# ThatTanishqTak/3D-Renderer

Hardware: AMD Instinct MI355X
Metric: frames/sec + Mpixels/sec at 1080p & 4K; achieved HBM GB/s vs roofline (higher is better)
Workload: dtype f32; 1 GPU; c3_grid1m_3840x2160; width=3840, height=2160, triangles=999698, vertices=501264, bin=32, skybox=reference Trident-Forge/Assets/Skyboxes PNG faces (512^2, assets/Skyboxes), frames_in_flight=3, parallelism=single GPU

## Files before the change

3d-renderer_amd/csrc/raster_bin.h:

```cpp
#pragma once
#include "raster_device.h"

#ifndef TRI_PK_SHADE
#error "raster_bin.h: define TRI_PK_SHADE (0 or 1) before the include"
#endif

#ifndef TRI_BIG_AREA
#define TRI_BIG_AREA 96
#endif
#ifndef TRI_BIG_AREA16
#define TRI_BIG_AREA16 160
#endif
#ifndef TRI_RASTER_PRIO
#define TRI_RASTER_PRIO 0
#endif
#ifndef TRI_QTAB_BIGN
#define TRI_QTAB_BIGN 192
#endif

namespace {

constexpr uint64_t kBgKey = 0x3F800001ull << 32;
constexpr float kPi = 3.14159265359f;

// ... 204 lines not shown
    cx0 = max(-floor_shift8(128 - xmin), ox);
    cx1 = min(floor_shift8(xmax - 128), ox + bw - 1);
    cy0 = max(-floor_shift8(128 - ymin), oy);
    cy1 = min(floor_shift8(ymax - 128), oy + bh - 1);
}

__device__ __forceinline__ uint32_t key_low(uint32_t prim_sub) {
    return ((TRI_PRIM_MAX - (prim_sub >> 3)) << 3) | (prim_sub & 7u);
}

constexpr uint32_t kQtab = 256, kQPrimMax = (1u << 20) - 1u;
__device__ __forceinline__ uint32_t qenc(uint32_t prim_sub, uint32_t qpos) {
    const uint32_t low = ((kQPrimMax - (prim_sub >> 3)) << 11) | ((prim_sub & 7u) << 8) | qpos;
    return (TRI_PRIM_MAX - (low >> 3)) << 3 | (low & 7u);
}

__device__ __forceinline__ bool edge_start(const TriRec& r, int32_t cx0, int32_t cy0, int32_t A[3], int32_t B[3],
                                          int32_t F[3], float& dzdX, float& dzdY) {
    const int32_t xmin = min(r.X[0], min(r.X[1], r.X[2])), xmax = max(r.X[0], max(r.X[1], r.X[2]));
    const int32_t ymin = min(r.Y[0], min(r.Y[1], r.Y[2])), ymax = max(r.Y[0], max(r.Y[1], r.Y[2]));
    if (xmax - xmin < 16384 && ymax - ymin < 16384) {
        const int32_t Xc = 256 * cx0 + 128, Yc = 256 * cy0 + 128;
#pragma unroll
        for (int k = 0; k < 3; ++k) {
            const int i = k, j = (k + 1) % 3;
            const int32_t a = r.Y[i] - r.Y[j];
            const int32_t bb = r.X[j] - r.X[i];
            const bool tl = (a > 0) || (a == 0 && bb > 0);
            A[k] = a;
            B[k] = bb;
// ... 697 lines not shown
    const uint4 &st = sh.st, &sd = sh.sd, &ss = sh.ss;
    TriTexDesc td;
    td.texels = reinterpret_cast<const uint32_t*>(((uint64_t)sd.y << 32) | sd.x);
    td.w = sd.z; td.h = sd.w;
    td.solid[0] = __uint_as_float(ss.x); td.solid[1] = __uint_as_float(ss.y);
    td.solid[2] = __uint_as_float(ss.z); td.solid[3] = __uint_as_float(ss.w);
    const float4 tx = (kAblate & 128) ? make_float4(u, v, u, 1.0f) : sample_tex(td, u, v, lut);
    const float4 tint = make_float4(__uint_as_float(st.x), __uint_as_float(st.y), __uint_as_float(st.z), __uint_as_float(st.w));
    put(11, tx.x); put(12, tx.y); put(13, tx.z); put(14, tx.w);
    put(15, tint.x); put(16, tint.y); put(17, tint.z); put(18, tint.w);
}

template <bool EXACT, bool SHADOW, bool ONE, int CLIPM = 0, int KIND = kKindGeneric, typename Put>
__device__ __forceinline__ void fetch_fragment_to(const TriFrameParams& fp, const TriDeviceBuffers& b, uint64_t key,
                                                  int32_t px, int32_t py, const float* lut, Put&& put,
                                                  const uint32_t* qtab = nullptr, const FetchBufs* fbk = nullptr) {
    constexpr bool kInlineVis = SHADOW;
    const uint32_t low = (uint32_t)key;
    const uint32_t prim = qtab ? kQPrimMax - (low >> 11) : TRI_PRIM_MAX - (low >> 3);
    const uint32_t sub = CLIPM == 1 ? 0u : (qtab ? (low >> 8) & 7u : low & 7u);
    const FetchBufs fb = (KIND >= 0 && fbk) ? *fbk : fetch_bufs<ONE, KIND>(fp, b);
    constexpr bool kEarly = ONE && !EXACT && !SHADOW;
    const bool ucol = ONE && kind_flag<KIND>(TRI_KIND_UCOL, obj_mode(fp) && fp.obj_ucol);
    const bool vcol = KIND >= 0 ? !ucol : (kEarly || !ucol);
    uint32_t sl[3] = {0, 0, 0}, d = 0;
    TriSnap a0{}, a1{}, a2{};
    uint32_t v0 = 0, v1 = 0, v2 = 0, dl = 0;
    Taps taps;
    if (CLIPM != 2) {
        if (qtab) {
            const uint32_t q = low & 0xFFu;
            sl[0] = qtab[q]; sl[1] = qtab[kQtab + q]; sl[2] = qtab[2 * kQtab + q];
            if (!ONE) d = qtab[3 * kQtab + q];
        } else {
            prim_slots<ONE, !SHADOW>(fp, b, prim, sl, d);
// ... 41 lines not shown

    float vis = 1.0f;
    if constexpr (kInlineVis && !(kAblate & 2048)) {
        auto ix = [&](uint32_t a, uint32_t bq, uint32_t c) {
            return interp_exact(w0, w1, w2, __uint_as_float(a), __uint_as_float(bq), __uint_as_float(c));
        };
        vis = shadow_vis(fp, b.shadow_map, ix(L0.x, L1.x, L2.x), ix(L0.y, L1.y, L2.y), ix(L0.z, L1.z, L2.z));
    }
    put(19, vis);
    fetch_attrs<EXACT, ONE, !SHADOW, KIND>(fp, b, fb, taps, d, w0, w1, w2, lut, put);
}

template <bool EXACT, bool SHADOW, bool ONE, int CLIPM = 0, int KIND = kKindGeneric>
__device__ __forceinline__ void fetch_fragment(const TriFrameParams& fp, const TriDeviceBuffers& b, uint64_t key,
                                               int32_t px, int32_t py, const float* lut, Frag& f,
                                               const uint32_t* qtab = nullptr, const FetchBufs* fbk = nullptr) {
    fetch_fragment_to<EXACT, SHADOW, ONE, CLIPM, KIND>(fp, b, key, px, py, lut, [&](int i, float x) { (&f.wx)[i] = x; },
                                                       qtab, fbk);
}

template <bool FAST = false>
__device__ __forceinline__ int cube_face(f3 d, float& s, float& t) {
    const float ax = fabsf(d.x), ay = fabsf(d.y), az = fabsf(d.z);
    int face;
    float ma, sc, tc;
    if (ax >= ay && ax >= az) {
        face = d.x >= 0.0f ? 0 : 1; ma = ax; sc = d.x >= 0.0f ? -d.z : d.z; tc = -d.y;
    } else if (ay >= az) {
        face = d.y >= 0.0f ? 2 : 3; ma = ay; sc = d.x; tc = d.y >= 0.0f ? d.z : -d.z;
    } else {
        face = d.z >= 0.0f ? 4 : 5; ma = az; sc = d.z >= 0.0f ? d.x : -d.x; tc = -d.y;
    }
    if (!(ma > 0.0f)) { s = 0.5f; t = 0.5f; return face; }
// ... 213 lines not shown
        const float w = fp.ai_wgt;
        const float alpha = ONE ? fp.sc.sbt[3] : c.w;
        if (fs_fast_nan(fp.sc, f)) return unorm8(mix_ai(alpha, ai.w, w)) << 24;
        return fast_bgra(mix_ai(c.x, 255.0f * ai.x, w), mix_ai(c.y, 255.0f * ai.y, w), mix_ai(c.z, 255.0f * ai.z, w),
                         unorm8(mix_ai(alpha, ai.w, w)));
    }
    return fast_bgra(c.x, c.y, c.z, ONE ? a8 : unorm8(c.w));
}

template <bool EXACT, int BL, bool SHADOW, bool ONE = false, bool AI = false, int KIND = kKindGeneric>
__device__ __forceinline__ void raster_bin(const TriFrameParams& fp, const TriDeviceBuffers& b, const int bin) {
    constexpr int BIN = 1 << BL;
    __shared__ uint64_t keys[BIN * BIN];
    constexpr bool kBalanced = BL == 4;
    constexpr bool kQt = BL == 5 && (ONE || SHADOW);
    constexpr uint32_t kQw = ONE ? 3u : 4u;
    constexpr int kBigN = kBalanced ? kBigQueue / 2 : ((kQt && ONE) ? TRI_QTAB_BIGN : kBigQueue);
    __shared__ uint32_t bigq[kBigN];
    __shared__ float lut[512];
    constexpr int kJobWords = (kBalanced && kCovJobs > BIN * BIN ? kCovJobs : BIN * BIN);
    __shared__ uint16_t skyq[kJobWords];
    __shared__ CovEntry cov[kBalanced ? kCovPass : 1];
    __shared__ uint32_t wsum[TRI_BLOCK / 64];
    __shared__ uint32_t nbig, nsky;
    __shared__ uint32_t qtab[kQt ? kQw * kQtab : 1];
    __shared__ uint16_t bigqp[kQt ? kBigN : 1];
    const int tid = threadIdx.x;
    TRI_STAMP(0);
    if constexpr (BL == 5) __builtin_amdgcn_s_setprio(1 + TRI_RASTER_PRIO);
    const int bx = bin % fp.nbx, by = bin / fp.nbx;
    const int32_t ox = bx * BIN, oy = fp.y0 + by * BIN;
    const int32_t bw = min(BIN, fp.W - ox), bh = min(BIN, fp.y1 - oy);
    const uint32_t cnt_v = __builtin_amdgcn_raw_buffer_load_b32(make_rsrc(b.bin_count, 4ull * fp.nbins), (uint32_t)bin * 4u, 0, 0);
    uint32_t pre1 = 0;
    if constexpr (!kBalanced) {
        const Rsrc qr = make_rsrc(b.bin_list + (size_t)bin * fp.bin_cap, 4ull * fp.bin_cap);
        pre1 = __builtin_amdgcn_raw_buffer_load_b32(qr, (uint32_t)tid * 4u, 0, 0);
    }
    for (int i = tid; i < BIN * BIN; i += TRI_BLOCK) keys[i] = kBgKey;
    if (fp.need_lut)
        for (int i = tid; i < 512; i += TRI_BLOCK) lut[i] = b.srgb_lut[i];
    if (tid == 0) {
        nbig = 0;
        nsky = 0;
    }
    lds_barrier();
    TRI_STAMP(1);
    const uint32_t cnt = (uint32_t)__builtin_amdgcn_readfirstlane((int)cnt_v);
    const uint32_t* queue = b.bin_list + (size_t)bin * fp.bin_cap;
    uint32_t s0 = 0, s1 = min(cnt, fp.bin_cap);
    const bool qmode = kQt && cnt <= kQtab && fp.nprims <= kQPrimMax;
    if (kAblate & 2) {
        if (s1 > s0) {
            const TriRec r = load_entry<ONE, !SHADOW>(fp, b, queue[0]);
            const uint64_t key = (0x3F000000ull << 32) | key_low(r.prim_sub);
            for (int i = tid; i < BIN * BIN; i += TRI_BLOCK) keys[i] = key;
        }
        s1 = s0;
    }
// ... 56 lines not shown
        const uint32_t njobs = min(total, (uint32_t)kCovJobs);
        for (uint32_t j = tid; j < njobs; j += TRI_BLOCK) {
            const uint32_t jb = jobs[j];
            cov_row<BL>(cov[jb >> 6], jb & 63u, keys);
        }
        for (uint32_t k = (start < (uint32_t)kCovJobs ? (uint32_t)kCovJobs - start : 0u); k < nrows; ++k)
            cov_row<BL>(cov[tid], k, keys);
        __syncthreads();
    }
  } else {
    auto cover = [&](uint32_t i, int32_t sub, int32_t step, bool first) {
        const uint32_t ri = first ? pre1 : queue[i];
        uint32_t dq;
        TriRec r = load_entry_d<ONE, !SHADOW>(fp, b, ri, dq);
        if (kQt && qmode) {
            if (!(ri & TRI_ENTRY_CLIPPED)) {
                qtab[i] = r.v[0]; qtab[kQtab + i] = r.v[2]; qtab[2 * kQtab + i] = r.v[1];
                if (!ONE) qtab[3 * kQtab + i] = dq;
            }
            r.prim_sub = qenc(r.prim_sub, i);
        }
        int32_t cx0, cx1, cy0, cy1;
        rec_bbox(r, ox, oy, bw, bh, cx0, cx1, cy0, cy1);
        if (cx0 > cx1 || cy0 > cy1) return;
        if ((cx1 - cx0 + 1) * (cy1 - cy0 + 1) > big_area<BL>()) {
            if (sub != 0) return;
            const uint32_t q = atomicAdd(&nbig, 1u);
            if (q < (uint32_t)kBigN) {
                bigq[q] = ri;
                if (kQt) bigqp[q] = (uint16_t)i;
                return;
            }
            raster_serial<BL>(r, cx0, cx1, cy0, cy1, ox, oy, keys);
            return;
        }
        raster_span<BL>(r, cx0, cx1, cy0, cy1, ox, oy, keys, sub, step);
    };
    for (uint32_t i = s0 + tid; i < s1; i += TRI_BLOCK) cover(i, 0, 1, i < (uint32_t)TRI_BLOCK);
    __syncthreads();
// ... 58 lines not shown
    };
    auto store_z = [&](size_t o, uint32_t o32, float z) {
        if (!write_depth) return;
        if constexpr (KIND >= 0) *(TRI_G float*)(dbase + o32) = z;
        else b.depth[o] = z;
    };
    const uint32_t bg_sgpr = sky_const ? fp.sky_bgra : fp.clear_bgra;
    auto bg_bgra = [&]() {
        uint32_t v = bg_sgpr;
        asm volatile("" : "+s"(v));
        return v;
    };
    constexpr bool kDefer = BL <= 5;
    static_assert(!kQt || kDefer, "the queue-position table holds no clipped entry: their pixels must be deferred");
    constexpr int kWaveQ = BIN * BIN / (TRI_BLOCK / 64);
    __shared__ uint16_t clipq[kDefer ? BIN * BIN : 1];
    uint32_t nclip = 0;
    auto shade_loop = [&](auto QT) {
        constexpr bool kq = decltype(QT)::value;
        if constexpr (KIND >= 0) __builtin_amdgcn_s_waitcnt(0x0F70);
        uint32_t so_it = so - so_step;
        for (int ly = tid >> BL; ly < bh; ly += TRI_BLOCK / BIN) {
            so_it += so_step;
            const bool in = lx < bw;
            const uint64_t key = in ? keys[(ly << BL) + lx] : 0ull;
            const bool bg = in && key == kBgKey;
            if constexpr (kDefer) {
                const bool clipped = in && !bg && (((uint32_t)key >> (kq ? 8 : 0)) & 7u) != 0u;
                const uint64_t m = __ballot(clipped);
                if (m) {
                    if (clipped) clipq[(tid >> 6) * kWaveQ + nclip + lanes_below(m)] = (uint16_t)((ly << BL) + lx);
                    nclip += (uint32_t)__builtin_popcountll(m);
                }
                if (clipped) continue;
            }
            if (sky_queue) {
                const uint64_t m = __ballot(bg);
                if (m) {
                    const uint32_t lane = lanes_below(~0ull);
                    const uint32_t leader = (uint32_t)__builtin_ctzll(m);
                    uint32_t base = 0;
                    if (lane == leader) base = atomicAdd(&nsky, (uint32_t)__builtin_popcountll(m));
                    base = (uint32_t)__builtin_amdgcn_readlane((int)base, (int)leader);
                    if (bg) skyq[base + lanes_below(m)] = (uint16_t)((ly << BL) + lx);
                }
            }
// ... 24 lines not shown
            float z;
            if (bg) {
                const size_t o = KIND >= 0 ? 0 : (size_t)(py - fp.y0) * fp.W + px;
                if (!sky_queue) store_c(o, so_it, bg_bgra());
                store_z(o, so_it, 1.0f);
                continue;
            } else if (kAblate & 1) {
                z = __uint_as_float((uint32_t)(key >> 32));
                out = (uint32_t)key;
            } else {
                z = __uint_as_float((uint32_t)(key >> 32));
                Frag f;
                if (kAblate & 256) {
                    const float k0 = __uint_as_float(((uint32_t)key & 0x7FFFFFu) | 0x3F000000u);
                    for (int q = 0; q < 20; ++q) (&f.wx)[q] = k0 + 0.01f * q;
                } else {
                    fetch_fragment<EXACT, SHADOW, ONE, kDefer ? 1 : 0, KIND>(fp, b, key, px, py, lut, f, kq ? qtab : nullptr, &fbk);
                }
                out = shade_bgra<EXACT, ONE, AI, KIND>(fp, b, f, px, py, npt_k);
            }
            const size_t o = KIND >= 0 ? 0 : (size_t)(py - fp.y0) * fp.W + px;
            store_c(o, so_it, out);
            store_z(o, so_it, z);
        }
    };
    if (kQt && qmode) shade_loop(std::true_type{});
    else shade_loop(std::false_type{});
    if constexpr (kDefer) {
        __builtin_amdgcn_wave_barrier();
        for (uint32_t i = (uint32_t)(tid & 63); i < nclip; i += 64) {
            const uint32_t li = clipq[(tid >> 6) * kWaveQ + i];
            const int32_t qx = (int32_t)(li & (BIN - 1)), qy = (int32_t)(li >> BL);
            const uint64_t key = keys[li];
            const int32_t px = ox + qx, py = oy + qy;
            Frag f;
            fetch_fragment<EXACT, SHADOW, ONE, 2, KIND>(fp, b, key, px, py, lut, f, (kQt && qmode) ? qtab : nullptr, &fbk);
            const size_t o = (size_t)(py - fp.y0) * fp.W + px;
            const uint32_t o32 = KIND >= 0 ? (uint32_t)((py - fp.y0) * fp.W + px) * 4u : 0u;
            store_c(o, o32, shade_bgra<EXACT, ONE, AI, KIND>(fp, b, f, px, py, npt_k));
            store_z(o, o32, __uint_as_float((uint32_t)(key >> 32)));
        }
    }
#ifdef TRI_PHASE_TIMING
    __syncthreads();
    TRI_STAMP(4);
    if (!sky_queue || fp.sky_mode == TRI_SKY_PREFILLED) { TRI_STAMP(5); return; }
#endif
    if (!sky_queue || fp.sky_mode == TRI_SKY_PREFILLED) return;
    __syncthreads();
    const uint32_t ns = nsky;
    if (fp.sky_lut && !fp.need_lut && ns > 0) {
        for (int i = tid; i < 512; i += TRI_BLOCK) lut[i] = b.srgb_lut[i];
        __syncthreads();
    }
    const bool persp = !EXACT && fp.sky_mode == TRI_SKY_PERSP;
    for (uint32_t i = tid; i < ns; i += TRI_BLOCK) {
        const uint32_t li = skyq[i];
        const int32_t px = ox + (int32_t)(li & (BIN - 1)), py = oy + (int32_t)(li >> BL);
        b.color[(size_t)(py - fp.y0) * fp.W + px] =
            persp ? sky_bgra_persp(fp, b, px, py, lut) : sky_bgra(fp, b, px, py, lut);
    }
#ifdef TRI_PHASE_TIMING
    __syncthreads();
    TRI_STAMP(5);
#endif
}

}
```

3d-renderer_amd/csrc/raster_common.h:

```cpp
#pragma once

#include <stdint.h>
#include "../../include/tri_raster.h"

#define TRI_BIN_LOG2 6
#define TRI_BIN (1 << TRI_BIN_LOG2)
#define TRI_BLOCK 256
#define TRI_PRIM_MAX ((1u << 29) - 1u)
#define TRI_ENTRY_CLIPPED 0x80000000u
#define TRI_PRIM_CLIPPED 0x80000000u
#define TRI_MAX_CLIP_VERTS 12
#define TRI_MAX_CLIP_POLY 9
static_assert(TRI_MAX_CLIP_POLY - 2 <= 7, "clipped sub-triangle number k = 1..nsub must fit 3 bits");
static_assert(TRI_MAX_CLIP_POLY <= TRI_MAX_CLIP_VERTS, "clip polygon buffers");
#define TRI_WMIN 1e-5f
#define TRI_GUARD_BAND_PX 16000.0f
#ifndef TRI_MAX_PPT
#define TRI_MAX_PPT 16
#endif
#define TRI_OBJ48_DRAWS 16

#define TRI_SKY_RAY 0u
#define TRI_SKY_PERSP 1u
#define TRI_SKY_UNIFORM 2u
// ... 78 lines not shown
struct __attribute__((aligned(16))) TriDrawShade {
    float tint[4];
    TriTexDesc tex;
};
static_assert(sizeof(TriDrawShade) == 48, "TriDrawShade: tint + texture descriptor");

struct TriCounters {
    uint32_t ovf_records;
    uint32_t ovf_verts;
    uint32_t tris_setup;
    uint32_t tris_clipped;
    uint32_t bin_entries;
    uint32_t sbin_max;
    uint32_t bin_max;
    uint32_t flags;
};

struct TriShadeConst {
    float cam[4];
    float base[4];
    float metallic, roughness, amb_strength;
    float om;
    float amb[4];
    uint32_t has_sun, npt;
    uint32_t a8;
    float kd;
    float sun_l[4];
    float sun_rad[4];
    struct {
        float pos[4];
// ... 55 lines not shown
```

3d-renderer_amd/csrc/raster_launch.h:

```cpp
#pragma once

#include <hip/hip_runtime.h>
#include <vector>
#include "raster_common.h"

#ifndef TRI_SETUP_WAVES
#define TRI_SETUP_WAVES 6
#endif
#ifndef TRI_SETUP_WGS_PER_CU
#define TRI_SETUP_WGS_PER_CU TRI_SETUP_WAVES
#endif

#if defined(__HIP_DEVICE_COMPILE__) && defined(TRI_KERNEL_TU)
#define TRI_G __attribute__((address_space(1)))
#else
#define TRI_G
#endif

struct TriDeviceBuffers {
    TRI_G const TriVsIn* vin;
    TRI_G const float* vpos;
    TRI_G const float* vattr;
    TRI_G const TriVsSkin* vskin;
    TRI_G const float* bones;
// ... 111 lines not shown
    TRI_G uint32_t* resolved;
    TRI_G uint8_t* mask;
    uint32_t Wr, Hr, Wo, Ho, ndraws;
    float rx, ry, ox, oy;
    float sx, sy, hw, hh;
    float alpha, jx, jy;
    uint32_t has_prev, reject_id;
};
hipError_t tri_launch_upscale_resolve(const TriUpscaleArgs& args, hipStream_t stream);
const void* tri_id_raster_kernel(const TriFrameParams& fp);
#ifdef TRI_DIAG_FRONT
void tri_diag_front_plan(TriFramePlan& plan);
#endif
const void* tri_raster_plain_kernel(const TriFrameParams& fp);
int tri_raster_kind(const TriFrameParams& fp);
enum TriFrontKernel { kFrontVertex = 0, kFrontBand, kFrontReset };
const void* tri_vertex_stage_kernel(TriFrontKernel k);

enum TriStage { kStageVertex = 0, kStageShadow, kStageSetup, kStageRaster, kStageCount };

hipError_t tri_run_plan(const TriFramePlan& plan, const TriLaunchArgs& args, TriLaunchArgs* d_args,
                        hipStream_t stream, hipEvent_t* events, const TriIdArgs* id = nullptr,
                        hipEvent_t* id_events = nullptr, const TriMotionArgs* motion = nullptr,
                        hipEvent_t* motion_events = nullptr);

hipError_t tri_launch_id_collect(const uint32_t* ids, int32_t W, int32_t x0, int32_t row0, int32_t w, int32_t h,
                                 uint32_t* bits, uint32_t nwords, hipStream_t stream);
hipError_t tri_launch_id_outline(const uint32_t* ids, const uint32_t* sel, uint32_t ndraws, uint32_t* color, int32_t W,
                                 int32_t rows, int32_t r, const float rgba[4], hipStream_t stream);

// ... 92 lines not shown
```

3d-renderer_amd/csrc/raster_plain.hip:

```cpp
#define TRI_KERNEL_TU 1
#define TRI_PK_SHADE 0
#include "raster_bin.h"

#ifndef TRI_RASTER_WAVES_PLAIN
#define TRI_RASTER_WAVES_PLAIN 7
#endif
#ifndef TRI_RASTER_WAVES_PLAIN_ONE
#define TRI_RASTER_WAVES_PLAIN_ONE 8
#endif
#ifndef TRI_RASTER_ONE_VGPRS
#define TRI_RASTER_ONE_VGPRS 28
#endif
#ifndef TRI_KIND_WAVES
#define TRI_KIND_WAVES 8
#endif
#ifndef TRI_KIND_VGPRS
#define TRI_KIND_VGPRS 32
#endif

namespace {

template <bool EXACT, int BL, bool ONE>
__global__ __launch_bounds__(TRI_BLOCK) __attribute__((amdgpu_waves_per_eu(BL <= 5 ? ((ONE && !EXACT) ? TRI_RASTER_WAVES_PLAIN_ONE : TRI_RASTER_WAVES_PLAIN) : 3))) void k_raster_plain(TRI_KARGS) {
    TRI_BIND_ARGS;
// ... 7 lines not shown
}
#endif
#if TRI_KIND_VGPRS
#define TRI_KIND_VGPR_ATTR __attribute__((amdgpu_num_vgpr(TRI_KIND_VGPRS)))
#else
#define TRI_KIND_VGPR_ATTR
#endif
#define TRI_KIND_KERNEL(NAME, BL, ATTR, KIND)                                                                      \
    __global__ __launch_bounds__(TRI_BLOCK) ATTR void NAME(TRI_KARGS) {                                            \
        TRI_BIND_ARGS;                                                                                             \
        raster_bin<false, BL, false, true, false, (int)(KIND)>(fp, b, xcd_bin(blockIdx.x, fp.nbins));              \
    }
#define TRI_KIND_ATTR5 __attribute__((amdgpu_waves_per_eu(TRI_KIND_WAVES))) TRI_KIND_VGPR_ATTR
#define TRI_KIND_ATTR4 __attribute__((amdgpu_waves_per_eu(TRI_RASTER_WAVES_PLAIN_ONE)))
constexpr uint32_t kKindLit = TRI_KIND_SUN | TRI_KIND_LIGHTS | TRI_KIND_DEPTH;
TRI_KIND_KERNEL(k_raster_kind5_lit_sky, 5, TRI_KIND_ATTR5, kKindLit | TRI_KIND_SKYQ)
TRI_KIND_KERNEL(k_raster_kind5_lit_sky_xf, 5, TRI_KIND_ATTR5, kKindLit | TRI_KIND_SKYQ | TRI_KIND_XFORM)
TRI_KIND_KERNEL(k_raster_kind5_lit, 5, TRI_KIND_ATTR5, kKindLit)
TRI_KIND_KERNEL(k_raster_kind4_ucol_pl_sky, 4, TRI_KIND_ATTR4, TRI_KIND_UCOL | TRI_KIND_LIGHTS | TRI_KIND_DEPTH | TRI_KIND_SKYQ)
template <bool EXACT, int BL>
__global__ __launch_bounds__(TRI_BLOCK) __attribute__((amdgpu_waves_per_eu(BL <= 5 ? TRI_RASTER_WAVES_PLAIN : 3))) void k_raster_ai(TRI_KARGS) {
    TRI_BIND_ARGS;
    raster_bin<EXACT, BL, false, false, true>(fp, b, xcd_bin(blockIdx.x, fp.nbins));
}

const void* kind_kernel(int bl, uint32_t kind) {
    auto f = [](auto kernel) { return reinterpret_cast<const void*>(kernel); };
    if (bl == 5) {
        if (kind == (kKindLit | TRI_KIND_SKYQ)) return f(k_raster_kind5_lit_sky);
        if (kind == (kKindLit | TRI_KIND_SKYQ | TRI_KIND_XFORM)) return f(k_raster_kind5_lit_sky_xf);
        if (kind == kKindLit) return f(k_raster_kind5_lit);
    }
    if (bl == 4 && kind == (TRI_KIND_UCOL | TRI_KIND_LIGHTS | TRI_KIND_DEPTH | TRI_KIND_SKYQ)) return f(k_raster_kind4_ucol_pl_sky);
    return nullptr;
}

template <int BL>
const void* plain_kernel(bool exact, bool one, bool ai) {
    auto f = [](auto kernel) { return reinterpret_cast<const void*>(kernel); };
    if (ai) return exact ? f(k_raster_ai<true, BL>) : f(k_raster_ai<false, BL>);
    if (one) return exact ? f(k_raster_plain<true, BL, true>) : f(k_raster_plain<false, BL, true>);
    return exact ? f(k_raster_plain<true, BL, false>) : f(k_raster_plain<false, BL, false>);
}

}

int tri_raster_kind(const TriFrameParams& fp) {
    if (!(fp.one_draw && fp.shade_solid && fp.vary_obj) || fp.exact_shading || fp.ai_on || fp.shadow_on) return -1;
    if ((uint64_t)fp.W * (uint64_t)(fp.y1 - fp.y0) * 4ull >= (1ull << 32)) return -1;
    const bool sky_on = fp.sky_size != 0;
    const uint32_t kind = (fp.obj_xform ? TRI_KIND_XFORM : 0u) | (fp.obj_ucol ? TRI_KIND_UCOL : 0u) |
                          (fp.sc.has_sun ? TRI_KIND_SUN : 0u) | (fp.write_depth ? TRI_KIND_DEPTH : 0u) |
                          (sky_on && fp.sky_mode != TRI_SKY_UNIFORM ? TRI_KIND_SKYQ : 0u) |
                          (fp.sc.npt ? TRI_KIND_LIGHTS : 0u);
    return kind_kernel(fp.bin_log2, kind) ? (int)kind : -1;
}
const void* tri_raster_plain_kernel(const TriFrameParams& fp) {
    const int kind = tri_raster_kind(fp);
    if (kind >= 0) return kind_kernel(fp.bin_log2, (uint32_t)kind);
    const bool exact = fp.exact_shading != 0, one = fp.one_draw && fp.shade_solid, ai = fp.ai_on != 0;
    return fp.bin_log2 == 5   ? plain_kernel<5>(exact, one, ai)
           : fp.bin_log2 == 4 ? plain_kernel<4>(exact, one, ai)
                              : plain_kernel<6>(exact, one, ai);
}
#ifdef TRI_PRIM_GROUPS
extern "C" int tri_debug_prim_groups(unsigned long long* out3, int reset) {
    if (reset) {
        const unsigned long long z[3] = {0, 0, 0};
        return hipMemcpyToSymbol(HIP_SYMBOL(g_tri_groups), z, sizeof(z)) == hipSuccess ? 0 : -1;
    }
    return hipMemcpyFromSymbol(out3, HIP_SYMBOL(g_tri_groups), 3 * sizeof(unsigned long long), 0,
// ... 10 lines not shown
```

3d-renderer_amd/csrc/tri_raster_capi.hip:

```cpp
#include "tri_ctx.h"

#include <chrono>
#include <string>

using fsel::unorm8_host;

namespace {

thread_local std::string g_last_error;

int upload_texture_table(tri_ctx* c) {
    if (!c->tex_dirty) return TRI_OK;
    TriTexDesc* h = c->texdesc;
    for (int s = 0; s < TRI_MAX_TEXTURE_SLOTS; ++s) {
        const int src = c->d_tex[s] ? s : 0;
        h[s].texels = c->d_tex[src];
        h[s].w = c->tex_w[src];
        h[s].h = c->tex_h[src];
        const uint32_t p = c->tex_solid[src];
        for (int k = 0; k < 3; ++k) h[s].solid[k] = fsel::srgb_decode((p >> (8 * k)) & 0xFF);
        h[s].solid[3] = (float)(p >> 24) / 255.0f;
    }
    c->need_lut = fsel::slots_need_lut(h);
    c->tex_dirty = false;
// ... 664 lines not shown
    for (const uint2& w : ws) {
        setup += w.x;
        entries += w.y;
    }
    out->triangles_setup = setup;
    out->triangles_clipped = h.tris_clipped;
    out->bin_entries = entries;
    out->vertices_shaded = c->res.nslots;
    out->bins_x = (uint32_t)c->nbx;
    out->bins_y = (uint32_t)c->nby;
    out->bin_size = 1u << c->bin_log2;
    out->path = c->last_path;
    return TRI_OK;
}

}
```

3d-renderer_amd/python/trident_raster/abi.py:

```python
import ctypes as C

import numpy as np

TRI_RASTER_ABI_VERSION = 2

TRI_OK = 0
TRI_E_INVALID = -1
TRI_E_HIP = -2
TRI_E_OOM = -3
TRI_E_OVERFLOW = -4
TRI_E_UNSUPPORTED = -5
TRI_E_STATE = -6
TRI_E_TIMEOUT = -7

TRI_MAX_POINT_LIGHTS = 8
TRI_MAX_TEXTURE_SLOTS = 256
TRI_FLAG_NO_DEPTH_OUTPUT = 0x1
TRI_FLAG_EXACT_SHADING = 0x2
TRI_FLAG_CLUSTER_CULL = 0x4

VERTEX_DTYPE = np.dtype(
    [
        ("position", "<f4", 3),
        ("normal", "<f4", 3),
# ... 433 lines not shown
    ("tri_animset_create", C.c_int, [C.c_int32, C.POINTER(C.c_void_p)]),
    ("tri_animset_destroy", C.c_int, [C.c_void_p]),
    ("tri_animset_add_skeleton", C.c_int, [C.c_void_p, C.c_void_p, C.c_uint32, C.c_int32, C.POINTER(C.c_uint32)]),
    ("tri_animset_add_clip", C.c_int, [C.c_void_p, C.c_uint32, C.c_void_p, C.c_uint32, C.c_void_p, C.c_void_p, C.c_uint32,
                                       C.c_void_p, C.c_void_p, C.c_uint32, C.c_float, C.POINTER(C.c_uint32)]),
    ("tri_pose_palette", C.c_int, [C.c_void_p, C.c_void_p, C.c_void_p, C.c_uint32]),
    ("tri_read_bone_palette", C.c_int, [C.c_void_p, C.c_void_p, C.c_uint32]),
    ("tri_group_pose_palette", C.c_int, [C.c_void_p, C.POINTER(C.c_void_p), C.c_void_p, C.c_uint32]),
    ("tri_animset_add_mask", C.c_int, [C.c_void_p, C.c_uint32, C.c_void_p, C.c_uint32, C.POINTER(C.c_uint32)]),
    ("tri_pose_graph", C.c_int, [C.c_void_p, C.c_void_p, C.c_void_p, C.c_uint32, C.c_void_p, C.c_uint32]),
    ("tri_group_pose_graph", C.c_int, [C.c_void_p, C.POINTER(C.c_void_p), C.c_void_p, C.c_uint32, C.c_void_p,
                                       C.c_uint32]),
    ("tri_set_timing", C.c_int, [C.c_void_p, C.c_int]),
    ("tri_get_timing", C.c_int, [C.c_void_p, C.POINTER(TriTiming)]),
    ("tri_get_frame_stats", C.c_int, [C.c_void_p, C.POINTER(TriFrameStats)]),
    ("tri_set_shadow", C.c_int, [C.c_void_p, C.POINTER(TriShadowConfig)]),
    ("tri_shadow_fit_ortho", C.c_int, [C.POINTER(C.c_float * 3), C.POINTER(C.c_float * 3), C.POINTER(C.c_float * 3),
                                       C.POINTER(C.c_float * 16)]),
    ("tri_read_shadow_map", C.c_int, [C.c_void_p, C.c_void_p]),
    ("tri_get_output", C.c_int, [C.c_void_p, C.POINTER(TriImage)]),
    ("tri_geometry_create", C.c_int, [C.c_int32, C.POINTER(C.c_void_p)]),
    ("tri_geometry_upload", C.c_int,
     [C.c_void_p, C.c_void_p, C.c_uint64, C.c_void_p, C.c_uint64, C.c_void_p, C.c_uint32]),
    ("tri_geometry_destroy", C.c_int, [C.c_void_p]),
    ("tri_bind_geometry", C.c_int, [C.c_void_p, C.c_void_p]),
    ("tri_group_create", C.c_int, [C.POINTER(TriGroupConfig), C.POINTER(C.c_void_p)]),
    ("tri_group_destroy", C.c_int, [C.c_void_p]),
    ("tri_group_context", C.c_int, [C.c_void_p, C.c_uint32, C.POINTER(C.c_void_p)]),
    ("tri_group_upload_geometry", C.c_int,
     [C.c_void_p, C.c_void_p, C.c_uint64, C.c_void_p, C.c_uint64, C.c_void_p, C.c_uint32]),
# ... 99 lines not shown
```

3d-renderer_amd/python/trident_raster/raster.py:

```python
import ctypes as C
import os

import numpy as np

from . import abi

_HERE = os.path.dirname(os.path.abspath(__file__))
PKG_ROOT = os.path.normpath(os.path.join(_HERE, "..", ".."))
LIB_PATH = os.path.join(PKG_ROOT, "lib", "libtri_raster.so")

_lib = None


class TriError(RuntimeError):
    def __init__(self, code, msg):
        super().__init__(f"tri_raster error {code}: {msg}")
        self.code = code


def load_library(path=None):
    global _lib
    if _lib is not None:
        return _lib
    path = path or os.environ.get("TRI_RASTER_LIB") or LIB_PATH
# ... 282 lines not shown
        return ms.value, n.value

    def set_timing(self, enable, period=1):
        _check(_lib.tri_set_timing(self._ctx, int(period) if enable else 0))

    def timing(self):
        t = abi.TriTiming()
        _check(_lib.tri_get_timing(self._ctx, C.byref(t)))
        return {k: getattr(t, k) for k, _ in abi.TriTiming._fields_}

    def frame_stats(self):
        s = abi.TriFrameStats()
        _check(_lib.tri_get_frame_stats(self._ctx, C.byref(s)))
        return {k: getattr(s, k) for k, _ in abi.TriFrameStats._fields_}


def _motion_history(prev_view, prev_projection, prev_models, draw_count=None):
    h = abi.TriMotionHistory()
    h.prev_view = (C.c_float * 16)(*np.asarray(prev_view, np.float32).reshape(16).tolist())
    h.prev_projection = (C.c_float * 16)(*np.asarray(prev_projection, np.float32).reshape(16).tolist())
    m = None
    if prev_models is not None:
        m = np.ascontiguousarray(prev_models, dtype=np.float32).reshape(-1, 16)
        h.prev_models = m.ctypes.data_as(C.POINTER(C.c_float))
        h.draw_count = m.shape[0]
    if draw_count is not None:
        h.draw_count = int(draw_count)
    return h, m


# ... 760 lines not shown
```

include/tri_raster.h:

```cpp
#ifndef TRI_RASTER_H
#define TRI_RASTER_H

#include <stddef.h>
#include <stdint.h>

#ifdef __cplusplus
extern "C" {
#endif

#define TRI_RASTER_ABI_VERSION 2

#define TRI_OK 0
#define TRI_E_INVALID (-1)
#define TRI_E_HIP (-2)
#define TRI_E_OOM (-3)
#define TRI_E_OVERFLOW (-4)
#define TRI_E_UNSUPPORTED (-5)
#define TRI_E_STATE (-6)
#define TRI_E_TIMEOUT (-7)

#define TRI_MAX_POINT_LIGHTS 8
#define TRI_MAX_TEXTURE_SLOTS 256
#define TRI_MAX_BONE_INFLUENCES 4
#define TRI_MAX_DIM 8192
// ... 489 lines not shown
int tri_xfer_frame(tri_xfer* xfer, uint32_t slot, tri_ctx* ctx, void* depth, const tri_global_ubo* ubo,
                   const float clear_rgba[4], const tri_draw* draws, uint32_t draw_count, uint32_t exchange);
int tri_xfer_synchronize(tri_xfer* xfer);
int tri_xfer_wait(tri_xfer* xfer);
int tri_xfer_set_timeout(tri_xfer* xfer, uint32_t timeout_ms);
int tri_xfer_comm_count(tri_xfer* xfer, uint32_t* count);
int tri_xfer_info(tri_xfer* xfer, uint64_t* sent_bytes, uint64_t* received_bytes, uint32_t* max_slot_bytes);
typedef struct tri_xfer_loopback tri_xfer_loopback;
int tri_xfer_loopback_create(uint32_t world, tri_xfer_loopback** out);
int tri_xfer_loopback_destroy(tri_xfer_loopback* hub);
int tri_xfer_comm_create_loopback(tri_xfer_loopback* hub, uint32_t rank, int32_t device, tri_xfer_comm** out);

int tri_set_timing(tri_ctx* ctx, int enable);
int tri_get_timing(tri_ctx* ctx, tri_timing* out);
int tri_get_frame_stats(tri_ctx* ctx, tri_frame_stats* out);

typedef struct tri_group tri_group;
typedef struct tri_group_config {
    uint32_t width;
    uint32_t height;
    uint32_t device_count;
    uint32_t display;
    const int32_t* devices;
    uint32_t flags;
    uint32_t group_flags;
} tri_group_config;
#define TRI_GROUP_NO_PACK 0x1u
#define TRI_GROUP_STAGE_BANDS 0x2u
#define TRI_GROUP_PACK_BGR24 0x4u
#define TRI_GROUP_FMT_BGRA32 0u
// ... 67 lines not shown
```

Baseline: 11340 frames/s.

## Stage per-bin vertex attributes in an LDS hash table for fast lit kernels

During binning, each non-clipped queued triangle inserts its three vertex slots into a shared-memory open-addressing hash table. The owning thread loads the vertex's snapped position, inverse w and varyings into LDS, and the queue table then stores packed bucket indices. Shading then reads vertex data from LDS instead of gathering from global memory per pixel, which aims to cut redundant vertex fetches where triangles are tiny and share vertices. Bins whose table overflows fall back to the gather path. The cost is extra atomics and LDS use (the sRGB LUT region is reused), a smaller big-triangle queue, and an added device counter.

```diff
diff --git a/3d-renderer_amd/csrc/raster_bin.h b/3d-renderer_amd/csrc/raster_bin.h
--- a/3d-renderer_amd/csrc/raster_bin.h
+++ b/3d-renderer_amd/csrc/raster_bin.h
@@ -242,6 +242,12 @@
     const uint32_t low = ((kQPrimMax - (prim_sub >> 3)) << 11) | ((prim_sub & 7u) << 8) | qpos;
     return (TRI_PRIM_MAX - (low >> 3)) << 3 | (low & 7u);
 }
+
+constexpr int kKindStage = 1 << 16;
+constexpr uint32_t kVtBuckets = 144, kVtProbe = 24, kVtEmpty = 0xFFFFFFFFu;
+constexpr int kVtBigN = 32;
+template <int KIND, int BL>
+constexpr bool vstage_kind() { return BL == 5 && KIND >= 0 && (KIND & kKindStage) != 0; }
 
 __device__ __forceinline__ bool edge_start(const TriRec& r, int32_t cx0, int32_t cy0, int32_t A[3], int32_t B[3],
                                           int32_t F[3], float& dzdX, float& dzdY) {
@@ -969,11 +975,13 @@
 template <bool EXACT, bool SHADOW, bool ONE, int CLIPM = 0, int KIND = kKindGeneric, typename Put>
 __device__ __forceinline__ void fetch_fragment_to(const TriFrameParams& fp, const TriDeviceBuffers& b, uint64_t key,
                                                   int32_t px, int32_t py, const float* lut, Put&& put,
-                                                  const uint32_t* qtab = nullptr, const FetchBufs* fbk = nullptr) {
+                                                  const uint32_t* qtab = nullptr, const FetchBufs* fbk = nullptr,
+                                                  bool qprim = false) {
     constexpr bool kInlineVis = SHADOW;
     const uint32_t low = (uint32_t)key;
-    const uint32_t prim = qtab ? kQPrimMax - (low >> 11) : TRI_PRIM_MAX - (low >> 3);
-    const uint32_t sub = CLIPM == 1 ? 0u : (qtab ? (low >> 8) & 7u : low & 7u);
+    const bool qk = qtab || qprim;
+    const uint32_t prim = qk ? kQPrimMax - (low >> 11) : TRI_PRIM_MAX - (low >> 3);
+    const uint32_t sub = CLIPM == 1 ? 0u : (qk ? (low >> 8) & 7u : low & 7u);
     const FetchBufs fb = (KIND >= 0 && fbk) ? *fbk : fetch_bufs<ONE, KIND>(fp, b);
     constexpr bool kEarly = ONE && !EXACT && !SHADOW;
     const bool ucol = ONE && kind_flag<KIND>(TRI_KIND_UCOL, obj_mode(fp) && fp.obj_ucol);
@@ -1045,9 +1053,35 @@
 template <bool EXACT, bool SHADOW, bool ONE, int CLIPM = 0, int KIND = kKindGeneric>
 __device__ __forceinline__ void fetch_fragment(const TriFrameParams& fp, const TriDeviceBuffers& b, uint64_t key,
                                                int32_t px, int32_t py, const float* lut, Frag& f,
-                                               const uint32_t* qtab = nullptr, const FetchBufs* fbk = nullptr) {
+                                               const uint32_t* qtab = nullptr, const FetchBufs* fbk = nullptr,
+                                               bool qprim = false) {
     fetch_fragment_to<EXACT, SHADOW, ONE, CLIPM, KIND>(fp, b, key, px, py, lut, [&](int i, float x) { (&f.wx)[i] = x; },
-                                                       qtab, fbk);
+                                                       qtab, fbk, qprim);
+}
+
+template <int KIND>
+__device__ __forceinline__ void fetch_fragment_staged(const TriFrameParams& fp, const TriDeviceBuffers& b, uint64_t key,
+                                                      int32_t px, int32_t py, const uint32_t* qtab, const V4* vtab,
+                                                      const FetchBufs& fbk, Frag& f) {
+    const uint32_t w = qtab[(uint32_t)key & 0xFFu];
+    const V4* r0 = vtab + 3u * (w & 0xFFu);
+    const V4* r1 = vtab + 3u * ((w >> 8) & 0xFFu);
+    const V4* r2 = vtab + 3u * ((w >> 16) & 0xFFu);
+    const V4 p0 = r0[0], p1 = r0[1], p2 = r0[2];
+    const V4 q0 = r1[0], q1 = r1[1], q2 = r1[2];
+    const V4 s0 = r2[0], s1 = r2[1], s2 = r2[2];
+    const TriSnap a0{__float_as_int(p0.x), __float_as_int(p0.y), p0.z, 0.0f};
+    const TriSnap a1{__float_as_int(q0.x), __float_as_int(q0.y), q0.z, 0.0f};
+    const TriSnap a2{__float_as_int(s0.x), __float_as_int(s0.y), s0.z, 0.0f};
+    float w0, w1, w2;
+    fast_weights_snaps(a0, a1, a2, px, py, w0, w1, w2);
+    Taps t;
+    t.a0 = V4{p0.w, p1.x, p1.y, 0.0f}; t.a1 = V4{p1.z, p1.w, p2.x, 0.0f}; t.a2 = V4{p2.y, p2.z, p2.w, 0.0f};
+    t.b0 = V4{s0.w, s1.x, s1.y, 0.0f}; t.b1 = V4{s1.z, s1.w, s2.x, 0.0f}; t.b2 = V4{s2.y, s2.z, s2.w, 0.0f};
+    t.c0 = V4{q0.w, q1.x, q1.y, 0.0f}; t.c1 = V4{q1.z, q1.w, q2.x, 0.0f}; t.c2 = V4{q2.y, q2.z, q2.w, 0.0f};
+    auto put = [&](int i, float x) { (&f.wx)[i] = x; };
+    put(19, 1.0f);
+    fetch_attrs<false, true, true, KIND>(fp, b, fbk, t, 0u, w0, w1, w2, nullptr, put);
 }
 
 template <bool FAST = false>
@@ -1291,10 +1325,21 @@
     __shared__ uint64_t keys[BIN * BIN];
     constexpr bool kBalanced = BL == 4;
     constexpr bool kQt = BL == 5 && (ONE || SHADOW);
-    constexpr uint32_t kQw = ONE ? 3u : 4u;
-    constexpr int kBigN = kBalanced ? kBigQueue / 2 : ((kQt && ONE) ? TRI_QTAB_BIGN : kBigQueue);
+    constexpr bool kVs = vstage_kind<KIND, BL>();
+    static_assert(kVtBuckets == 144u && kVtBuckets <= 256u, "the probe steps are coprime to 144; a bucket number is a byte");
+    static_assert(!kVs || (ONE && !EXACT && !SHADOW && !AI), "the vertex table: the fast single-draw kinds only");
+    constexpr uint32_t kQw = kVs ? 1u : (ONE ? 3u : 4u);
+    constexpr int kBigN = kBalanced ? kBigQueue / 2 : (kVs ? kVtBigN : ((kQt && ONE) ? TRI_QTAB_BIGN : kBigQueue));
     __shared__ uint32_t bigq[kBigN];
-    __shared__ float lut[512];
+    __shared__ float lut[kVs ? 1 : 512];
+    __shared__ V4 vtab[kVs ? 3 * kVtBuckets : 1];
+    __shared__ uint32_t vs_fail;
+    __shared__ uint32_t clipq_vs[kVs ? BIN * BIN / 2 : 1];
+    auto lutp = [&]() -> float* {
+        if constexpr (kVs) return reinterpret_cast<float*>(vtab);
+        else return lut;
+    };
+    uint32_t* const vtag = clipq_vs;
     constexpr int kJobWords = (kBalanced && kCovJobs > BIN * BIN ? kCovJobs : BIN * BIN);
     __shared__ uint16_t skyq[kJobWords];
     __shared__ CovEntry cov[kBalanced ? kCovPass : 1];
@@ -1315,11 +1360,16 @@
         pre1 = __builtin_amdgcn_raw_buffer_load_b32(qr, (uint32_t)tid * 4u, 0, 0);
     }
     for (int i = tid; i < BIN * BIN; i += TRI_BLOCK) keys[i] = kBgKey;
-    if (fp.need_lut)
-        for (int i = tid; i < 512; i += TRI_BLOCK) lut[i] = b.srgb_lut[i];
+    if constexpr (kVs) {
+        if (tid < (int)kVtBuckets) vtag[tid] = kVtEmpty;
+    } else {
+        if (fp.need_lut)
+            for (int i = tid; i < 512; i += TRI_BLOCK) lut[i] = b.srgb_lut[i];
+    }
     if (tid == 0) {
         nbig = 0;
         nsky = 0;
+        if constexpr (kVs) vs_fail = 0;
     }
     lds_barrier();
     TRI_STAMP(1);
@@ -1406,7 +1456,7 @@
         uint32_t dq;
         TriRec r = load_entry_d<ONE, !SHADOW>(fp, b, ri, dq);
         if (kQt && qmode) {
-            if (!(ri & TRI_ENTRY_CLIPPED)) {
+            if (!kVs && !(ri & TRI_ENTRY_CLIPPED)) {
                 qtab[i] = r.v[0]; qtab[kQtab + i] = r.v[2]; qtab[2 * kQtab + i] = r.v[1];
                 if (!ONE) qtab[3 * kQtab + i] = dq;
             }
@@ -1415,6 +1465,40 @@
         int32_t cx0, cx1, cy0, cy1;
         rec_bbox(r, ox, oy, bw, bh, cx0, cx1, cy0, cy1);
         if (cx0 > cx1 || cy0 > cy1) return;
+        if constexpr (kVs) {
+            if (qmode && !(ri & TRI_ENTRY_CLIPPED)) {
+                const FetchBufs fbc = fetch_bufs<ONE, KIND>(fp, b);
+                const int vo[3] = {0, 2, 1};
+                uint32_t word = 0;
+#pragma unroll
+                for (int k = 0; k < 3; ++k) {
+                    const uint32_t slot = r.v[vo[k]];
+                    const uint32_t quo = slot / kVtBuckets;
+                    uint32_t h = slot - quo * kVtBuckets;
+                    const uint32_t step = 6u * (quo & 3u) + 1u + (quo & 4u);
+                    bool own = false, ok = false;
+#pragma unroll 1
+                    for (uint32_t t = 0; t < kVtProbe; ++t) {
+                        const uint32_t old = atomicCAS(&vtag[h], kVtEmpty, slot);
+                        own = old == kVtEmpty;
+                        ok = own || old == slot;
+                        if (ok) break;
+                        h = h + step >= kVtBuckets ? h + step - kVtBuckets : h + step;
+                    }
+                    if (!ok) vs_fail = 1u;
+                    word |= h << (8 * k);
+                    if (own) {
+                        const V4 p = ld_vary<true, true>(fbc, slot, 0), n = ld_vary<true, true>(fbc, slot, 1),
+                                 c = ld_vary<true, true>(fbc, slot, 2);
+                        V4* rec = vtab + 3u * h;
+                        rec[0] = V4{(float)r.X[vo[k]], (float)r.Y[vo[k]], r.iw[vo[k]], p.x};
+                        rec[1] = V4{p.y, p.z, n.x, n.y};
+                        rec[2] = V4{n.z, c.x, c.y, c.z};
+                    }
+                }
+                qtab[i] = word;
+            }
+        }
         if ((cx1 - cx0 + 1) * (cy1 - cy0 + 1) > big_area<BL>()) {
             if (sub != 0) return;
             const uint32_t q = atomicAdd(&nbig, 1u);
@@ -1503,10 +1587,20 @@
     constexpr bool kDefer = BL <= 5;
     static_assert(!kQt || kDefer, "the queue-position table holds no clipped entry: their pixels must be deferred");
     constexpr int kWaveQ = BIN * BIN / (TRI_BLOCK / 64);
-    __shared__ uint16_t clipq[kDefer ? BIN * BIN : 1];
+    __shared__ uint16_t clipq[(kDefer && !kVs) ? BIN * BIN : 1];
+    auto clipq_at = [&](uint32_t i) -> uint16_t& {
+        if constexpr (kVs) return reinterpret_cast<uint16_t*>(clipq_vs)[i];
+        else return clipq[i];
+    };
     uint32_t nclip = 0;
+    bool staged = false;
+    if constexpr (kVs) {
+        staged = qmode && __builtin_amdgcn_readfirstlane((int)vs_fail) == 0;
+        if (tid == 0 && cnt != 0u) atomicAdd(staged ? &b.counters->vs_staged : &b.counters->vs_fallback, 1u);
+    }
     auto shade_loop = [&](auto QT) {
-        constexpr bool kq = decltype(QT)::value;
+        constexpr int kqm = (int)decltype(QT)::value;
+        constexpr bool kq = kqm != 0;
         if constexpr (KIND >= 0) __builtin_amdgcn_s_waitcnt(0x0F70);
         uint32_t so_it = so - so_step;
         for (int ly = tid >> BL; ly < bh; ly += TRI_BLOCK / BIN) {
@@ -1518,7 +1612,7 @@
                 const bool clipped = in && !bg && (((uint32_t)key >> (kq ? 8 : 0)) & 7u) != 0u;
                 const uint64_t m = __ballot(clipped);
                 if (m) {
-                    if (clipped) clipq[(tid >> 6) * kWaveQ + nclip + lanes_below(m)] = (uint16_t)((ly << BL) + lx);
+                    if (clipped) clipq_at((tid >> 6) * kWaveQ + nclip + lanes_below(m)) = (uint16_t)((ly << BL) + lx);
                     nclip += (uint32_t)__builtin_popcountll(m);
                 }
                 if (clipped) continue;
@@ -1573,8 +1667,11 @@
                 if (kAblate & 256) {
                     const float k0 = __uint_as_float(((uint32_t)key & 0x7FFFFFu) | 0x3F000000u);
                     for (int q = 0; q < 20; ++q) (&f.wx)[q] = k0 + 0.01f * q;
+                } else if constexpr (kqm == 2) {
+                    fetch_fragment_staged<KIND>(fp, b, key, px, py, qtab, vtab, fbk, f);
                 } else {
-                    fetch_fragment<EXACT, SHADOW, ONE, kDefer ? 1 : 0, KIND>(fp, b, key, px, py, lut, f, kq ? qtab : nullptr, &fbk);
+                    fetch_fragment<EXACT, SHADOW, ONE, kDefer ? 1 : 0, KIND>(fp, b, key, px, py, lutp(), f,
+                                                                             kqm == 1 ? qtab : nullptr, &fbk, kqm == 3);
                 }
                 out = shade_bgra<EXACT, ONE, AI, KIND>(fp, b, f, px, py, npt_k);
             }
@@ -1583,17 +1680,24 @@
             store_z(o, so_it, z);
         }
     };
-    if (kQt && qmode) shade_loop(std::true_type{});
-    else shade_loop(std::false_type{});
+    if constexpr (kVs) {
+        if (staged) shade_loop(std::integral_constant<int, 2>{});
+        else if (qmode) shade_loop(std::integral_constant<int, 3>{});
+        else shade_loop(std::integral_constant<int, 0>{});
+    } else {
+        if (kQt && qmode) shade_loop(std::true_type{});
+        else shade_loop(std::false_type{});
+    }
     if constexpr (kDefer) {
         __builtin_amdgcn_wave_barrier();
         for (uint32_t i = (uint32_t)(tid & 63); i < nclip; i += 64) {
-            const uint32_t li = clipq[(tid >> 6) * kWaveQ + i];
+            const uint32_t li = clipq_at((tid >> 6) * kWaveQ + i);
             const int32_t qx = (int32_t)(li & (BIN - 1)), qy = (int32_t)(li >> BL);
             const uint64_t key = keys[li];
             const int32_t px = ox + qx, py = oy + qy;
             Frag f;
-            fetch_fragment<EXACT, SHADOW, ONE, 2, KIND>(fp, b, key, px, py, lut, f, (kQt && qmode) ? qtab : nullptr, &fbk);
+            fetch_fragment<EXACT, SHADOW, ONE, 2, KIND>(fp, b, key, px, py, lutp(), f,
+                                                        (kQt && !kVs && qmode) ? qtab : nullptr, &fbk, kVs && qmode);
             const size_t o = (size_t)(py - fp.y0) * fp.W + px;
             const uint32_t o32 = KIND >= 0 ? (uint32_t)((py - fp.y0) * fp.W + px) * 4u : 0u;
             store_c(o, o32, shade_bgra<EXACT, ONE, AI, KIND>(fp, b, f, px, py, npt_k));
@@ -1608,8 +1712,8 @@
     if (!sky_queue || fp.sky_mode == TRI_SKY_PREFILLED) return;
     __syncthreads();
     const uint32_t ns = nsky;
-    if (fp.sky_lut && !fp.need_lut && ns > 0) {
-        for (int i = tid; i < 512; i += TRI_BLOCK) lut[i] = b.srgb_lut[i];
+    if (fp.sky_lut && (kVs || !fp.need_lut) && ns > 0) {
+        for (int i = tid; i < 512; i += TRI_BLOCK) lutp()[i] = b.srgb_lut[i];
         __syncthreads();
     }
     const bool persp = !EXACT && fp.sky_mode == TRI_SKY_PERSP;
@@ -1617,7 +1721,7 @@
         const uint32_t li = skyq[i];
         const int32_t px = ox + (int32_t)(li & (BIN - 1)), py = oy + (int32_t)(li >> BL);
         b.color[(size_t)(py - fp.y0) * fp.W + px] =
-            persp ? sky_bgra_persp(fp, b, px, py, lut) : sky_bgra(fp, b, px, py, lut);
+            persp ? sky_bgra_persp(fp, b, px, py, lutp()) : sky_bgra(fp, b, px, py, lutp());
     }
 #ifdef TRI_PHASE_TIMING
     __syncthreads();
diff --git a/3d-renderer_amd/csrc/raster_common.h b/3d-renderer_amd/csrc/raster_common.h
--- a/3d-renderer_amd/csrc/raster_common.h
+++ b/3d-renderer_amd/csrc/raster_common.h
@@ -116,6 +116,7 @@
     uint32_t sbin_max;
     uint32_t bin_max;
     uint32_t flags;
+    uint32_t vs_staged, vs_fallback;
 };
 
 struct TriShadeConst {
diff --git a/3d-renderer_amd/csrc/raster_launch.h b/3d-renderer_amd/csrc/raster_launch.h
--- a/3d-renderer_amd/csrc/raster_launch.h
+++ b/3d-renderer_amd/csrc/raster_launch.h
@@ -149,6 +149,7 @@
 #endif
 const void* tri_raster_plain_kernel(const TriFrameParams& fp);
 int tri_raster_kind(const TriFrameParams& fp);
+void tri_raster_vertex_stage(bool on);
 enum TriFrontKernel { kFrontVertex = 0, kFrontBand, kFrontReset };
 const void* tri_vertex_stage_kernel(TriFrontKernel k);
 
diff --git a/3d-renderer_amd/csrc/raster_plain.hip b/3d-renderer_amd/csrc/raster_plain.hip
--- a/3d-renderer_amd/csrc/raster_plain.hip
+++ b/3d-renderer_amd/csrc/raster_plain.hip
@@ -45,8 +45,10 @@
 #define TRI_KIND_ATTR5 __attribute__((amdgpu_waves_per_eu(TRI_KIND_WAVES))) TRI_KIND_VGPR_ATTR
 #define TRI_KIND_ATTR4 __attribute__((amdgpu_waves_per_eu(TRI_RASTER_WAVES_PLAIN_ONE)))
 constexpr uint32_t kKindLit = TRI_KIND_SUN | TRI_KIND_LIGHTS | TRI_KIND_DEPTH;
-TRI_KIND_KERNEL(k_raster_kind5_lit_sky, 5, TRI_KIND_ATTR5, kKindLit | TRI_KIND_SKYQ)
-TRI_KIND_KERNEL(k_raster_kind5_lit_sky_xf, 5, TRI_KIND_ATTR5, kKindLit | TRI_KIND_SKYQ | TRI_KIND_XFORM)
+TRI_KIND_KERNEL(k_raster_kind5_lit_sky, 5, TRI_KIND_ATTR5, kKindLit | TRI_KIND_SKYQ | kKindStage)
+TRI_KIND_KERNEL(k_raster_kind5_lit_sky_xf, 5, TRI_KIND_ATTR5, kKindLit | TRI_KIND_SKYQ | TRI_KIND_XFORM | kKindStage)
+TRI_KIND_KERNEL(k_raster_kind5_lit_sky_gather, 5, TRI_KIND_ATTR5, kKindLit | TRI_KIND_SKYQ)
+TRI_KIND_KERNEL(k_raster_kind5_lit_sky_xf_gather, 5, TRI_KIND_ATTR5, kKindLit | TRI_KIND_SKYQ | TRI_KIND_XFORM)
 TRI_KIND_KERNEL(k_raster_kind5_lit, 5, TRI_KIND_ATTR5, kKindLit)
 TRI_KIND_KERNEL(k_raster_kind4_ucol_pl_sky, 4, TRI_KIND_ATTR4, TRI_KIND_UCOL | TRI_KIND_LIGHTS | TRI_KIND_DEPTH | TRI_KIND_SKYQ)
 template <bool EXACT, int BL>
@@ -55,11 +57,13 @@
     raster_bin<EXACT, BL, false, false, true>(fp, b, xcd_bin(blockIdx.x, fp.nbins));
 }
 
+bool g_vertex_stage = true;
 const void* kind_kernel(int bl, uint32_t kind) {
     auto f = [](auto kernel) { return reinterpret_cast<const void*>(kernel); };
     if (bl == 5) {
-        if (kind == (kKindLit | TRI_KIND_SKYQ)) return f(k_raster_kind5_lit_sky);
-        if (kind == (kKindLit | TRI_KIND_SKYQ | TRI_KIND_XFORM)) return f(k_raster_kind5_lit_sky_xf);
+        if (kind == (kKindLit | TRI_KIND_SKYQ)) return g_vertex_stage ? f(k_raster_kind5_lit_sky) : f(k_raster_kind5_lit_sky_gather);
+        if (kind == (kKindLit | TRI_KIND_SKYQ | TRI_KIND_XFORM))
+            return g_vertex_stage ? f(k_raster_kind5_lit_sky_xf) : f(k_raster_kind5_lit_sky_xf_gather);
         if (kind == kKindLit) return f(k_raster_kind5_lit);
     }
     if (bl == 4 && kind == (TRI_KIND_UCOL | TRI_KIND_LIGHTS | TRI_KIND_DEPTH | TRI_KIND_SKYQ)) return f(k_raster_kind4_ucol_pl_sky);
@@ -86,6 +90,7 @@
                           (fp.sc.npt ? TRI_KIND_LIGHTS : 0u);
     return kind_kernel(fp.bin_log2, kind) ? (int)kind : -1;
 }
+void tri_raster_vertex_stage(bool on) { g_vertex_stage = on; }
 const void* tri_raster_plain_kernel(const TriFrameParams& fp) {
     const int kind = tri_raster_kind(fp);
     if (kind >= 0) return kind_kernel(fp.bin_log2, (uint32_t)kind);
diff --git a/3d-renderer_amd/csrc/tri_raster_capi.hip b/3d-renderer_amd/csrc/tri_raster_capi.hip
--- a/3d-renderer_amd/csrc/tri_raster_capi.hip
+++ b/3d-renderer_amd/csrc/tri_raster_capi.hip
@@ -702,4 +702,22 @@
     return TRI_OK;
 }
 
-}
+int tri_get_vertex_stage_stats(tri_ctx* c, uint32_t* staged_bins, uint32_t* fallback_bins) {
+    if (!c || !staged_bins || !fallback_bins) return fail(TRI_E_INVALID, "tri_get_vertex_stage_stats: null argument");
+    int rc = make_current(c);
+    if (rc) return rc;
+    TRI_HIP_TRY(hipStreamSynchronize(c->stream));
+    uint32_t h[2];
+    TRI_HIP_TRY(hipMemcpy(h, &c->d_ctr->vs_staged, sizeof h, hipMemcpyDeviceToHost));
+    TRI_HIP_TRY(hipMemset(&c->d_ctr->vs_staged, 0, sizeof h));
+    *staged_bins = h[0];
+    *fallback_bins = h[1];
+    return TRI_OK;
+}
+
+int tri_set_vertex_stage(int enable) {
+    tri_raster_vertex_stage(enable != 0);
+    return TRI_OK;
+}
+
+}
diff --git a/3d-renderer_amd/python/trident_raster/abi.py b/3d-renderer_amd/python/trident_raster/abi.py
--- a/3d-renderer_amd/python/trident_raster/abi.py
+++ b/3d-renderer_amd/python/trident_raster/abi.py
@@ -471,6 +471,8 @@
     ("tri_set_timing", C.c_int, [C.c_void_p, C.c_int]),
     ("tri_get_timing", C.c_int, [C.c_void_p, C.POINTER(TriTiming)]),
     ("tri_get_frame_stats", C.c_int, [C.c_void_p, C.POINTER(TriFrameStats)]),
+    ("tri_get_vertex_stage_stats", C.c_int, [C.c_void_p, C.POINTER(C.c_uint32), C.POINTER(C.c_uint32)]),
+    ("tri_set_vertex_stage", C.c_int, [C.c_int]),
     ("tri_set_shadow", C.c_int, [C.c_void_p, C.POINTER(TriShadowConfig)]),
     ("tri_shadow_fit_ortho", C.c_int, [C.POINTER(C.c_float * 3), C.POINTER(C.c_float * 3), C.POINTER(C.c_float * 3),
                                        C.POINTER(C.c_float * 16)]),
diff --git a/3d-renderer_amd/python/trident_raster/raster.py b/3d-renderer_amd/python/trident_raster/raster.py
--- a/3d-renderer_amd/python/trident_raster/raster.py
+++ b/3d-renderer_amd/python/trident_raster/raster.py
@@ -320,6 +320,11 @@
         _check(_lib.tri_get_frame_stats(self._ctx, C.byref(s)))
         return {k: getattr(s, k) for k, _ in abi.TriFrameStats._fields_}
 
+    def vertex_stage_stats(self):
+        staged, fallback = C.c_uint32(0), C.c_uint32(0)
+        _check(_lib.tri_get_vertex_stage_stats(self._ctx, C.byref(staged), C.byref(fallback)))
+        return staged.value, fallback.value
+
 
 def _motion_history(prev_view, prev_projection, prev_models, draw_count=None):
     h = abi.TriMotionHistory()
diff --git a/include/tri_raster.h b/include/tri_raster.h
--- a/include/tri_raster.h
+++ b/include/tri_raster.h
@@ -527,6 +527,8 @@
 int tri_set_timing(tri_ctx* ctx, int enable);
 int tri_get_timing(tri_ctx* ctx, tri_timing* out);
 int tri_get_frame_stats(tri_ctx* ctx, tri_frame_stats* out);
+int tri_get_vertex_stage_stats(tri_ctx* ctx, uint32_t* staged_bins, uint32_t* fallback_bins);
+int tri_set_vertex_stage(int enable);
 
 typedef struct tri_group tri_group;
 typedef struct tri_group_config {
```

After: 10790 frames/s. 4.8% lower.
